# Rikorose/DeepFilterNet

Hardware: AMD Instinct MI355X
Metric: 48 kHz audio frames/sec (hop=480), DeepFilterNet3 enhance() (higher is better)
Workload: dtype f32 (storage and accumulation; GRU projections / recurrences, the fused DF-encoder convolutions and the pointwise halves of the ERB separable convolutions as fp16-split MFMAs: x = hi + lo in f16, hi*hi + hi*lo + lo*hi on v_mfma_f32_16x16x32_f16, ~2^-21 relative; see exact_fp32_ms_per_step); 1 GPU; DeepFilterNet3 (recalled shipped shape, conv_ch=64) enhance(pad=True), batch=256 clips x 10 s @48 kHz per GPU, 1002 STFT frames per clip; batch_per_gpu=256, global_batch=256, parallelism=clips sharded over 1 GPU(s); no collective, inputs_resident_in_hbm=True

## Files before the change

deepfilternet_amd/_lib.py:

```python
from __future__ import annotations

import ctypes as C
import os
from typing import Optional

import torch

_HERE = os.path.dirname(os.path.abspath(__file__))
DEFAULT_LIB = os.environ.get("DFX_LIBRARY") or os.path.join(_HERE, "csrc", "libdfx.so")

DFX_OK = 0
DFX_ERR_INVALID_ARG, DFX_ERR_UNSUPPORTED, DFX_ERR_HIP, DFX_ERR_NO_DEVICE, DFX_ERR_ALLOC = 1, 2, 3, 4, 5
_ERRNAMES = {1: "invalid argument", 2: "unsupported configuration", 3: "HIP runtime error", 4: "no HIP device",
             5: "allocation failed"}


class DfxError(RuntimeError):
    def __init__(self, code: int, msg: str):
        super().__init__(f"DF transform error: {msg} [{_ERRNAMES.get(code, code)}]")
        self.code = code


class ModelCfg(C.Structure):
    _fields_ = [(n, C.c_int32) for n in (
# ... 66 lines not shown
    "dfx_mf_filter": (_i, [_fp, _fp, _fp, _i, _i, _i, _i, _i, _i, _f, _f, _i64, _i64, _i, _i, _fp, _vp]),
    "dfx_pcm16_to_f32": (_i, [_vp, _i64, _fp, _vp]),
    "dfx_f32_to_pcm16": (_i, [_fp, _i64, _vp, _vp]),
    "dfx_resampler_create": (_i, [_i, _i, _i, C.c_double, _i, C.c_double, C.POINTER(_vp)]),
    "dfx_resampler_free": (None, [_vp]),
    "dfx_resampler_out_len": (_i64, [_vp, _i64]),
    "dfx_resampler_kernel": (_i, [_i, _i, _i, C.c_double, _i, C.c_double, C.POINTER(_i), C.POINTER(_i), C.POINTER(_i), _f32p, _i64]),
    "dfx_resample": (_i, [_vp, _fp, _i64, _i64, _i64, _fp, _i64, _vp]),
    "dfx_stream_create": (_i, [_vp, _vp, _i64, _i, C.POINTER(_vp)]),
    "dfx_stream_free": (None, [_vp]),
    "dfx_stream_reset": (_i, [_vp, _vp]),
    "dfx_stream_reset_streams": (_i, [_vp, C.POINTER(_i64), _i64, _vp]),
    "dfx_stream_frames": (_i, [_vp, C.POINTER(_i64)]),
    "dfx_stream_frame_length": (_i, [_vp]),
    "dfx_stream_delay_frames": (_i, [_vp]),
    "dfx_stream_set_atten_lim": (_i, [_vp, _f]),
    "dfx_stream_set_post_filter_beta": (_i, [_vp, _f]),
    "dfx_stream_set_channels": (_i, [_vp, _i, _i]),
    "dfx_stream_set_gating": (_i, [_vp, _i]),
    "dfx_stream_set_thresholds": (_i, [_vp, _f, _f, _f]),
    "dfx_stream_set_atten_lim_streams": (_i, [_vp, C.POINTER(_i64), _i64, C.POINTER(_f), _vp]),
    "dfx_stream_set_post_filter_beta_streams": (_i, [_vp, C.POINTER(_i64), _i64, C.POINTER(_f), _vp]),
    "dfx_stream_set_thresholds_streams": (_i, [_vp, C.POINTER(_i64), _i64, C.POINTER(_f), _vp]),
    "dfx_stream_get_settings": (_i, [_vp, C.POINTER(_f)]),
    "dfx_stream_process": (_i, [_vp, _fp, _i64, _fp, _fp, _vp]),
    "dfx_stream_set_pausable": (_i, [_vp, _i]),
    "dfx_stream_process_active": (_i, [_vp, _fp, _i64, _fp, _fp, _vp, _vp]),
    "dfx_stream_process_raw": (_i, [_vp, _fp, _fp, _fp, _vp, _fp, _vp]),
    "dfx_prof_kernel_count": (_i, []),
    "dfx_prof_kernel_name": (C.c_char_p, [_i]),
    "dfx_prof_enable": (_i, [C.c_uint32]),
    "dfx_prof_reset": (_i, []),
    "dfx_prof_read": (_i, [_i, C.POINTER(C.c_double), C.POINTER(_i64)]),
}

_LIB: Optional[C.CDLL] = None
_LIB_PATH: Optional[str] = None
_EMU = False


def _bind(lib: C.CDLL) -> None:
    missing = []
    for name, (res, args) in SIGNATURES.items():
        try:
            fn = getattr(lib, name)
        except AttributeError:
            missing.append(name)
            continue
        fn.restype, fn.argtypes = res, args
    if missing:
        raise RuntimeError(f"libdfx is missing symbols declared in include/dfx.h: {missing}")


def use_library(path: str) -> None:
    global _LIB, _LIB_PATH, _EMU
    lib = C.CDLL(path)
    _bind(lib)
    _LIB, _LIB_PATH = lib, path
    _EMU = bool(lib.dfx_is_emulator())


def lib() -> C.CDLL:
    if _LIB is None:
        if not os.path.exists(DEFAULT_LIB):
            from . import build as _build

# ... 81 lines not shown
```

deepfilternet_amd/csrc/dfx_common.h:

```cpp
#pragma once

#include "dfx_env.h"

#include <cstdarg>
#include <string>
#include <vector>

#include "dfx.h"

void dfx_set_error(const char *fmt, ...);
#define DFX_FAIL(code, ...)         \
    do {                            \
        dfx_set_error(__VA_ARGS__); \
        return (code);              \
    } while (0)
#define DFX_HIP(expr)                                                                                   \
    do {                                                                                                \
        hipError_t e__ = (expr);                                                                        \
        if (e__ != hipSuccess) DFX_FAIL(DFX_ERR_HIP, "%s failed: %s", #expr, hipGetErrorString(e__));   \
    } while (0)
#define DFX_LAUNCH_CHECK()                                                                              \
    do {                                                                                                \
        hipError_t e__ = hipGetLastError();                                                             \
        if (e__ != hipSuccess) DFX_FAIL(DFX_ERR_HIP, "kernel launch failed: %s", hipGetErrorString(e__)); \
    } while (0)
int dfx_require_device();

#define DFX_MAX_STAGES 12
struct DfxFftPlan {
    int N;
    int M;
    int nstage;
    int radix[DFX_MAX_STAGES];
};

struct dfx_bands {
    int nb = 0;
    int F = 0;
    std::vector<uint64_t> widths;
    int *d_start = nullptr;
    float *d_invw = nullptr;
// ... 81 lines not shown
```

deepfilternet_amd/csrc/dfx_gru_pair.h:

```cpp
#pragma once

#define DFX_GP_NW 4
#define DFX_GP_THREADS (64 * DFX_GP_NW)
#define DFX_GP_NS 2
#define DFX_GP_TILES (3 * DFX_GP_NS)
#define DFX_GP_NF (8 * DFX_GP_TILES)
#ifndef DFX_GP_FL
#define DFX_GP_FL 15
#endif
#define DFX_GP_FR (DFX_GP_NF - DFX_GP_FL)
#ifndef DFX_GP_PIN
#define DFX_GP_PIN 30
#endif
#ifndef DFX_GP_ABLATE
#define DFX_GP_ABLATE 0
#endif
#ifndef DFX_GP_TRACE
#define DFX_GP_TRACE 0
#endif
#if DFX_GP_TRACE
#define DFX_GP_TICK(i)                                                                  \
    do {                                                                                \
        unsigned long long now_;                                                        \
        asm volatile("s_memtime %0\n\ts_waitcnt lgkmcnt(0)" : "=s"(now_)::"memory");    \
        tk[i] += now_ - tlast;                                                          \
        tlast = now_;                                                                   \
    } while (0)
#else
#define DFX_GP_TICK(i) do { } while (0)
#endif
#define DFX_GP_ROWS 32
#define DFX_GP_SMEM_W ((size_t)DFX_GP_FL * DFX_GP_NW * 2 * 64 * 16)
#define DFX_GP_SMEM_H ((size_t)2 * DFX_GP_ROWS * DFX_GH_HROW * 2)
#define DFX_GP_SMEM (DFX_GP_SMEM_W + DFX_GP_SMEM_H + 64)
#define DFX_GP_POS_KC(f) ((f) / DFX_GP_TILES)
#define DFX_GP_POS_GATE(f) (((f) % DFX_GP_TILES) / DFX_GP_NS)
#define DFX_GP_POS_S(f) (((f) % DFX_GP_TILES) % DFX_GP_NS)
#define DFX_GP_POS_TILE(f) ((f) % DFX_GP_TILES)

struct DfxGpSched {
    int cls[DFX_GP_NF];
    int idx[DFX_GP_NF];
};
static constexpr DfxGpSched dfx_gp_make_sched() {
    DfxGpSched sc{};
    int nr = 0, nl = 0;
    for (int f = 0; f < DFX_GP_NF; ++f) {
        const bool lds = ((f + 1) * DFX_GP_FL / DFX_GP_NF) != (f * DFX_GP_FL / DFX_GP_NF);
        sc.cls[f] = lds ? 1 : 0;
        sc.idx[f] = lds ? nl++ : nr++;
    }
    return sc;
}

struct DfxGpSync {
    unsigned int *pflag = nullptr;
    unsigned int *pxcd = nullptr;
    unsigned int pbase = 0, tag = 0;
    int spin_limit = 1 << 22;
    unsigned int *err = nullptr;
    unsigned int *stat = nullptr;
    const unsigned int *ready = nullptr;
    unsigned int *done = nullptr;
    unsigned int base = 0;
    int K = 1;
    const int *tb = nullptr;
    unsigned long long *trace = nullptr;
    unsigned int *yprog = nullptr;
    const unsigned int *giprog[2] = {nullptr, nullptr};
    int sblk = 16, yblk = 16;
    unsigned int *xme = nullptr;
    const unsigned int *xprod[2] = {nullptr, nullptr};
    const unsigned int *xcons = nullptr;
    unsigned long long *ptrace = nullptr;
    int far = 0;
};

template <bool SEQ>
static __device__ __forceinline__ void dfx_gru_p2_run(const DfxGhArgs &A, int64_t pg, int half, const DfxGpSync &Y) {
    constexpr int H = 256, NF = DFX_GP_NF, HROW = DFX_GH_HROW, NW = DFX_GP_NW, NS = DFX_GP_NS, TILES = DFX_GP_TILES, ROWS = DFX_GP_ROWS;
    constexpr DfxGpSched SC = dfx_gp_make_sched();
    DFX_DYN_SMEM(unsigned char, smraw);
    dfx_h8 *wl = reinterpret_cast<dfx_h8 *>(smraw);
    uint16_t *h16 = reinterpret_cast<uint16_t *>(smraw + DFX_GP_SMEM_W);
    volatile int *sflag = reinterpret_cast<volatile int *>(smraw + DFX_GP_SMEM_W + DFX_GP_SMEM_H);
    const int tid = threadIdx.x, lane = tid & 63, wave = tid >> 6, q = lane >> 4, jl = lane & 15;
    const int64_t b0 = pg * ROWS;
    bool valid[2];
    int64_t brow[2];
#pragma unroll
    for (int n = 0; n < 2; ++n) {
        valid[n] = b0 + 16 * n + jl < A.B;
        brow[n] = valid[n] ? b0 + 16 * n + jl : A.B - 1;
    }
    const int ubase = 128 * half + 32 * wave;
    const dfx_h8 *wg = A.whf + lane;
#define DFX_GP_GIDX(f) (((((size_t)(8 * half + NS * wave + DFX_GP_POS_S(f))) * 8 + DFX_GP_POS_KC(f)) * 3 + DFX_GP_POS_GATE(f)) * 2 * 64)
    dfx_h8 wr[DFX_GP_FR][2];
    dfx_static_for<0, NF>([&](auto fc) {
        constexpr int f = decltype(fc)::value;
        if constexpr (SC.cls[f] == 0) {
            wr[SC.idx[f]][0] = wg[DFX_GP_GIDX(f)];
            wr[SC.idx[f]][1] = wg[DFX_GP_GIDX(f) + 64];
            if constexpr (SC.idx[f] < DFX_GP_PIN) {
                DFX_PIN_AGPR(wr[SC.idx[f]][0]);
                DFX_PIN_AGPR(wr[SC.idx[f]][1]);
            }
        } else {
            wl[((SC.idx[f] * NW + wave) * 2 + 0) * 64 + lane] = wg[DFX_GP_GIDX(f)];
            wl[((SC.idx[f] * NW + wave) * 2 + 1) * 64 + lane] = wg[DFX_GP_GIDX(f) + 64];
        }
    });
    float hp[2][NS][4];
    float4 bn[NS];
#pragma unroll
    for (int s = 0; s < NS; ++s) {
        bn[s] = *reinterpret_cast<const float4 *>(A.bhn + ubase + 16 * s + 4 * q);
#pragma unroll
        for (int n = 0; n < 2; ++n) hp[n][s][0] = hp[n][s][1] = hp[n][s][2] = hp[n][s][3] = 0.f;
    }
    auto put4 = [&](int row, int col, float v0, float v1, float v2, float v3) {
        const float v[4] = {v0, v1, v2, v3};
        uint16_t hh[4], hl[4];
#pragma unroll
        for (int r = 0; r < 4; ++r) {
            hh[r] = dfx_f32_to_f16_bits(v[r]);
            hl[r] = dfx_f32_to_f16_bits(v[r] - dfx_f16_bits_to_f32(hh[r]));
        }
        *reinterpret_cast<uint2 *>(h16 + ((size_t)0 * ROWS + row) * HROW + col) = make_uint2((uint32_t)hh[0] | ((uint32_t)hh[1] << 16), (uint32_t)hh[2] | ((uint32_t)hh[3] << 16));
        *reinterpret_cast<uint2 *>(h16 + ((size_t)1 * ROWS + row) * HROW + col) = make_uint2((uint32_t)hl[0] | ((uint32_t)hl[1] << 16), (uint32_t)hl[2] | ((uint32_t)hl[3] << 16));
    };
    for (int i = tid; i < (int)(DFX_GP_SMEM_H / 4); i += DFX_GP_THREADS) reinterpret_cast<uint32_t *>(h16)[i] = 0u;
    unsigned int *const fmine = Y.pflag + 16 * half;
    const unsigned int *const ftheirs = Y.pflag + 16 * (half ^ 1);
    bool dead = false;
    if (tid == 0) {
        const unsigned int me = Y.tag | (unsigned int)(dfx_xcc_id() + 1);
        __hip_atomic_store(Y.pxcd + half, me, __ATOMIC_RELAXED, __HIP_MEMORY_SCOPE_AGENT);
        if (Y.xme) __hip_atomic_store(Y.xme, me, __ATOMIC_RELAXED, __HIP_MEMORY_SCOPE_AGENT);
        unsigned int v;
        int spins = 0;
        while ((((v = __hip_atomic_load(Y.pxcd + (half ^ 1), __ATOMIC_RELAXED, __HIP_MEMORY_SCOPE_AGENT)) & ~15u) != Y.tag) || (v & 15u) == 0u) {
            if (++spins > Y.spin_limit) {
                dfx_raise(Y.err + 2);
                dead = true;
                break;
            }
            __builtin_amdgcn_s_sleep(2);
        }
        sflag[0] = (!dead && v == me && !Y.far) ? 1 : 0;
        sflag[1] = 0;
        if (Y.stat && half == 0 && v != me) __hip_atomic_fetch_add(Y.stat + 1, 1u, __ATOMIC_RELAXED, __HIP_MEMORY_SCOPE_AGENT);
    }
    __syncthreads();
    const bool light = sflag[0] != 0;
    const float *gp[2];
    float *yp[2];
    const float *ypo[4];
    const int prow = tid >> 3, pcol = 128 * (half ^ 1) + 4 * (tid & 7);
    {
        const int64_t r = b0 + prow < A.B ? b0 + prow : A.B - 1;
#pragma unroll
        for (int i = 0; i < 4; ++i) ypo[i] = A.y + r * A.T * H + pcol + 32 * i;
// ... 35 lines not shown
            }
            same = same && Y.xprod[i] && __hip_atomic_load(Y.xprod[i], __ATOMIC_RELAXED, __HIP_MEMORY_SCOPE_AGENT) == (Y.tag | (unsigned int)(dfx_xcc_id() + 1));
        }
        sflag[1] = same && !Y.far ? 1 : 0;
    };
#if DFX_GP_TRACE
    unsigned long long tk[12] = {0, 0, 0, 0, 0, 0, 0, 0, 0, 0, 0, 0}, tlast;
    asm volatile("s_memtime %0\n\ts_waitcnt lgkmcnt(0)" : "=s"(tlast)::"memory");
#endif
    const int nchunk = SEQ ? Y.K : 1;
    for (int ck = 0; ck < nchunk; ++ck) {
        const int64_t c0 = SEQ ? (int64_t)Y.tb[ck] : A.t0, c1 = SEQ ? (int64_t)Y.tb[ck + 1] : A.t1;
        if (SEQ) {
            if (tid == 0 && Y.trace) Y.trace[ck * 3 + 0] = wall_clock64();
            if (tid == 0 && !Y.giprog[0] && Y.ready) {
                const unsigned int want = Y.base + (unsigned int)ck + 1u;
                int spins = 0;
                while (!dead && (int)(__hip_atomic_load(Y.ready, __ATOMIC_RELAXED, __HIP_MEMORY_SCOPE_AGENT) - want) < 0) {
                    if (++spins > Y.spin_limit) {
                        dfx_raise(Y.err + 2);
                        dead = true;
                        break;
                    }
                    __builtin_amdgcn_s_sleep(8);
                }
            }
            if (tid == 0 && Y.giprog[0] && ck == 0) poll_gi(Y.sblk);
            __syncthreads();
            __builtin_amdgcn_fence(__ATOMIC_ACQUIRE, "agent");
            if (tid == 0 && Y.trace) Y.trace[ck * 3 + 1] = wall_clock64();
        }
        if (c1 > c0) load_gi(c0);
        for (int64_t t = c0; t < c1; ++t) {
            const unsigned char *hb = reinterpret_cast<const unsigned char *>(h16 + (size_t)jl * HROW + 8 * q);
            constexpr size_t HB_N = (size_t)16 * HROW * 2, HB_LO = (size_t)ROWS * HROW * 2, HB_KSTEP = 32 * 2;
            f32x4 acc[2][TILES];
#pragma unroll
            for (int n = 0; n < 2; ++n)
#pragma unroll
                for (int i = 0; i < TILES; ++i) acc[n][i] = f32x4{0.f, 0.f, 0.f, 0.f};
            dfx_h8 bh[2][2], bl[2][2];
#pragma unroll
            for (int n = 0; n < 2; ++n) {
                bh[0][n] = *reinterpret_cast<const dfx_h8 *>(hb + HB_N * n);
                bl[0][n] = *reinterpret_cast<const dfx_h8 *>(hb + HB_N * n + HB_LO);
            }
            dfx_h8 lhi[2][3], llo[2][3];
            dfx_static_for<0, 3>([&](auto ic) {
                constexpr int i = decltype(ic)::value;
                if constexpr (SC.cls[i] == 1) {
                    lhi[0][i] = wl[((SC.idx[i] * NW + wave) * 2 + 0) * 64 + lane];
                    llo[0][i] = wl[((SC.idx[i] * NW + wave) * 2 + 1) * 64 + lane];
                }
            });
            dfx_static_for<0, NF / 3>([&](auto gc) {
                constexpr int grp = decltype(gc)::value, f0 = 3 * grp;
                constexpr int kc = DFX_GP_POS_KC(f0);
                if constexpr (DFX_GP_POS_TILE(f0) == 0 && kc + 1 < 8) {
                    constexpr int kn = kc + 1;
#pragma unroll
                    for (int n = 0; n < 2; ++n) {
                        bh[kn & 1][n] = *reinterpret_cast<const dfx_h8 *>(hb + HB_N * n + HB_KSTEP * kn);
                        bl[kn & 1][n] = *reinterpret_cast<const dfx_h8 *>(hb + HB_N * n + HB_LO + HB_KSTEP * kn);
                    }
                }
                if constexpr (grp + 1 < NF / 3) {
                    dfx_static_for<0, 3>([&](auto ic) {
                        constexpr int i = decltype(ic)::value, f = f0 + 3 + i;
// ... 197 lines not shown
```

deepfilternet_amd/csrc/dfx_io.hip:

```cpp
#include <cmath>

#include "dfx_common.h"

#define DFX_RS_JT 16

struct dfx_resampler {
    int orig_sr = 0, new_sr = 0;
    int orig = 0, nw = 0, width = 0, K = 0, K4 = 0, nw_pad = 0;
    float *d_wt = nullptr;
    std::vector<float> w_host;
};

struct DfxRsArgs {
    int64_t B, T, x_stride, y_stride, out_len, frames;
    int orig, nw, nw_pad, width, K4, tn, fw, jw;
};

__global__ void __launch_bounds__(256) dfx_k_resample(const float *__restrict__ x, float *__restrict__ y, const float *__restrict__ wt,
                                                      DfxRsArgs A) {
    DFX_DYN_SMEM(float, xs);
    const int64_t tiles = (A.frames + A.tn - 1) / A.tn;
    const int64_t b = blockIdx.x / tiles;
    const int64_t n0 = (int64_t)(blockIdx.x - b * tiles) * A.tn;
    if (b >= A.B) return;
// ... 49 lines not shown
        out[i] = (float)in[i] * (1.0f / 32768.0f);
}
__global__ void dfx_k_f32_to_pcm16(const float *in, int64_t n, int16_t *out) {
    for (int64_t i = (int64_t)blockIdx.x * blockDim.x + threadIdx.x; i < n; i += (int64_t)gridDim.x * blockDim.x) {
        float v = in[i] * 32768.0f;
        v = v != v ? 0.f : fminf(fmaxf(v, -9.0e18f), 9.0e18f);
        out[i] = (int16_t)(uint16_t)(uint64_t)(int64_t)v;
    }
}

static unsigned io_grid(int64_t n) {
    const int64_t cap = (int64_t)dfx_env_num_cus() * 8, want = dfx_ceil_div(n, 256);
    return (unsigned)(want < cap ? (want > 0 ? want : 1) : cap);
}

extern "C" int dfx_pcm16_to_f32(const int16_t *pcm, int64_t n, float *out, void *stream) {
    if (n < 0) DFX_FAIL(DFX_ERR_INVALID_ARG, "dfx_pcm16_to_f32: bad arguments");
    if (int rc = dfx_require_device()) return rc;
    if (n == 0) return DFX_OK;
    if (!pcm || !out) DFX_FAIL(DFX_ERR_INVALID_ARG, "dfx_pcm16_to_f32: null buffer");
    DfxKScope ks(DFX_K_PCM, dfx_stream(stream));
    dfx_launch(dfx_k_pcm16_to_f32, dim3(io_grid(n)), dim3(256), 0, dfx_stream(stream), pcm, n, out);
    DFX_LAUNCH_CHECK();
    return DFX_OK;
}

extern "C" int dfx_f32_to_pcm16(const float *x, int64_t n, int16_t *out, void *stream) {
    if (n < 0) DFX_FAIL(DFX_ERR_INVALID_ARG, "dfx_f32_to_pcm16: bad arguments");
    if (int rc = dfx_require_device()) return rc;
    if (n == 0) return DFX_OK;
    if (!x || !out) DFX_FAIL(DFX_ERR_INVALID_ARG, "dfx_f32_to_pcm16: null buffer");
    DfxKScope ks(DFX_K_PCM, dfx_stream(stream));
    dfx_launch(dfx_k_f32_to_pcm16, dim3(io_grid(n)), dim3(256), 0, dfx_stream(stream), x, n, out);
    DFX_LAUNCH_CHECK();
    return DFX_OK;
}

static double bessel_i0(double x) {
    double sum = 1.0, term = 1.0;
    const double q = x * x / 4.0;
    for (int k = 1; k < 200; ++k) {
        term *= q / ((double)k * (double)k);
        sum += term;
        if (term < 1e-17 * sum) break;
    }
    return sum;
}

static int64_t gcd64(int64_t a, int64_t b) {
    while (b) {
        const int64_t t = a % b;
        a = b;
        b = t;
    }
    return a;
}

static int build_bank(dfx_resampler *r, int orig_sr, int new_sr, int lpw, double rolloff, int method, double beta) {
    if (orig_sr <= 0 || new_sr <= 0 || lpw <= 0 || rolloff <= 0.0 || rolloff > 1.0 || (method != 0 && method != 1))
        DFX_FAIL(DFX_ERR_INVALID_ARG, "dfx_resampler_create: bad arguments");
    const int64_t g = gcd64(orig_sr, new_sr);
    r->orig_sr = orig_sr, r->new_sr = new_sr;
    r->orig = (int)(orig_sr / g), r->nw = (int)(new_sr / g);
    const double base = (double)(r->orig < r->nw ? r->orig : r->nw) * rolloff;
    r->width = (int)std::ceil((double)lpw * r->orig / base);
    r->K = 2 * r->width + r->orig;
// ... 104 lines not shown
```

deepfilternet_amd/csrc/dfx_model.hip:

```cpp
#include "dfx_manifest.h"
#include "dfx_nn_kernels.h"

#include <cmath>
#include <functional>
#include <atomic>
#include <map>
#include <mutex>
#include <fcntl.h>
#include <sys/file.h>
#include <sys/stat.h>
#include <unistd.h>

static int check_cfg(const dfx_model_cfg *c) {
    if (!c) DFX_FAIL(DFX_ERR_INVALID_ARG, "null model cfg");
    if (c->conv_ch != 16 && c->conv_ch != 32 && c->conv_ch != 64)
        DFX_FAIL(DFX_ERR_UNSUPPORTED, "conv_ch=%d: the HIP kernels are instantiated for 16, 32, 64", c->conv_ch);
    if (c->emb_hidden_dim != 256 || c->df_hidden_dim != 256) DFX_FAIL(DFX_ERR_UNSUPPORTED, "GRU hidden size must be 256");
    if (c->nb_erb <= 0 || c->nb_erb % 8 || c->nb_erb > 64) DFX_FAIL(DFX_ERR_UNSUPPORTED, "nb_erb must be a multiple of 8, <= 64");
    if (c->nb_df <= 0 || c->nb_df % 2 || c->nb_df > c->fft_size / 2 + 1) DFX_FAIL(DFX_ERR_UNSUPPORTED, "nb_df must be even and <= F");
    if (c->df_order <= 0 || c->df_order > 16 || c->df_lookahead < 0 || c->df_lookahead >= c->df_order)
        DFX_FAIL(DFX_ERR_UNSUPPORTED, "need 0 <= df_lookahead < df_order <= 16");
    if (c->conv_lookahead < 0) DFX_FAIL(DFX_ERR_INVALID_ARG, "conv_lookahead < 0");
    if (c->emb_num_layers < 2 || c->df_num_layers < 1) DFX_FAIL(DFX_ERR_UNSUPPORTED, "emb_num_layers >= 2 and df_num_layers >= 1 required");
    if (c->df_pathway_kernel_size_t < 1 || c->df_pathway_kernel_size_t > 8) DFX_FAIL(DFX_ERR_UNSUPPORTED, "df_pathway_kernel_size_t must be 1..8");
// ... 1221 lines not shown
    w.gi = take(R * 768);
    w.xa2 = take(R * 256);
    w.xb2 = take(R * 256);
    w.gi2 = take(R * 768);
    w.demb = take(R * emb);
    w.d3 = take(R * (E / 4) * C);
    w.d2 = take(R * (E / 2) * C);
    w.d1 = take(R * E * C);
    w.mask = take(R * E);
    w.c0p = take(R * Fd * NO);
    w.xdf = take(R * 256);
    w.coefs = take(R * Fd * NO);
    w.lsnr = take(R);
    w.skp_e = take(c.emb_gru_skip_enc == DFX_SKIP_GROUPEDLINEAR ? R * emb : 0);
    w.skp_d = take(c.emb_gru_skip == DFX_SKIP_GROUPEDLINEAR ? R * emb : 0);
    const int nlayers = 1 + (c.emb_num_layers - 1) + c.df_num_layers;
    for (int l = 0; l < DFX_MAX_GRU_LAYERS; ++l) {
        const bool used = l < nlayers;
        w.pgi[l] = take(used ? R * 768 : 0);
        w.py[l] = take(used ? R * 256 : 0);
        w.ph[l] = take(used ? (B > 0 ? B : R) * 256 : 0);
    }
    w.total = off;
    return w;
}
}

extern "C" int dfx_model_workspace_bytes(const dfx_model *m, int64_t B, int64_t T, int64_t *bytes) {
    if (!m || !bytes || B < 0 || T < 0) DFX_FAIL(DFX_ERR_INVALID_ARG, "dfx_model_workspace_bytes: bad arguments");
    *bytes = (int64_t)(plan_ws(m->cfg, m->fuse_c0 && !m->c0_batch_unfused, B * T, B).total * sizeof(float)) + 256;
    return DFX_OK;
}

#include "dfx_model_launch.h"
#include "dfx_model_forward.h"
#include "dfx_model_stream.h"
#include "dfx_model_enhance.h"
```

deepfilternet_amd/csrc/dfx_nn_kernels.h:

```cpp
#pragma once

#include "dfx_common.h"

#include <type_traits>

#define DFX_ACT_NONE 0
#define DFX_ACT_RELU 1
#define DFX_ACT_TANH 2
#define DFX_ACT_SIGMOID 3

static __device__ __forceinline__ float dfx_sigmoid(float x) { return 1.f / (1.f + expf(-x)); }
static __device__ __forceinline__ float dfx_act(float v, int act) {
    if (act == DFX_ACT_RELU) return fmaxf(v, 0.f);
    if (act == DFX_ACT_TANH) return tanhf(v);
    if (act == DFX_ACT_SIGMOID) return dfx_sigmoid(v);
    return v;
}

template <int I, int N, typename F>
static __device__ __forceinline__ void dfx_static_for(F &&f) {
    if constexpr (I < N) {
        f(std::integral_constant<int, I>{});
        dfx_static_for<I + 1, N>(f);
    }
// ... 3884 lines not shown
    const dfx_h8 *wg = A.whf + lane;
#define DFX_GH_GIDX(f) (((((size_t)wave * NS + DFX_GH_POS_S(f)) * 8 + DFX_GH_POS_KC(f)) * 3 + DFX_GH_POS_GATE(f)) * 2 * 64)
    dfx_h8 wr[FR][2];
    dfx_static_for<0, NF>([&](auto fc) {
        constexpr int f = decltype(fc)::value;
        if constexpr (SC.cls[f] == 0) {
            wr[SC.idx[f]][0] = wg[DFX_GH_GIDX(f)];
            wr[SC.idx[f]][1] = wg[DFX_GH_GIDX(f) + 64];
            if constexpr (DFX_GH_PIN && !X32) {
                DFX_PIN_AGPR(wr[SC.idx[f]][0]);
                DFX_PIN_AGPR(wr[SC.idx[f]][1]);
            }
        } else if constexpr (SC.cls[f] == 1) {
            wl[((SC.idx[f] * NW + wave) * 2 + 0) * 64 + lane] = wg[DFX_GH_GIDX(f)];
            wl[((SC.idx[f] * NW + wave) * 2 + 1) * 64 + lane] = wg[DFX_GH_GIDX(f) + 64];
        }
    });
    float hp[NS][4];
    float4 bn[NS];
#pragma unroll
    for (int s = 0; s < NS; ++s) {
        const int u0 = UW * wave + 16 * s + 4 * q;
        bn[s] = *reinterpret_cast<const float4 *>(A.bhn + u0);
        float4 h0 = make_float4(0.f, 0.f, 0.f, 0.f);
        if (A.h_in) h0 = *reinterpret_cast<const float4 *>(A.h_in + brow * H + u0);
        hp[s][0] = h0.x, hp[s][1] = h0.y, hp[s][2] = h0.z, hp[s][3] = h0.w;
    }
    auto put_h16 = [&](int buf, int s) {
        if constexpr (X32) {
            *reinterpret_cast<float4 *>(h32 + ((size_t)buf * DFX_GH_ROWS + jl) * DFX_GH_HROW32 + UW * wave + 16 * s + 4 * q) =
                make_float4(hp[s][0], hp[s][1], hp[s][2], hp[s][3]);
            return;
        }
        uint16_t hh[4], hl[4];
#pragma unroll
        for (int r = 0; r < 4; ++r) {
            hh[r] = dfx_f32_to_f16_bits(hp[s][r]);
            hl[r] = dfx_f32_to_f16_bits(hp[s][r] - dfx_f16_bits_to_f32(hh[r]));
        }
        const int col = UW * wave + 16 * s + 4 * q;
        uint16_t *ph = h16 + ((size_t)(buf * 2 + 0) * DFX_GH_ROWS + jl) * HROW + col;
        uint16_t *pl = h16 + ((size_t)(buf * 2 + 1) * DFX_GH_ROWS + jl) * HROW + col;
        *reinterpret_cast<uint2 *>(ph) = make_uint2((uint32_t)hh[0] | ((uint32_t)hh[1] << 16), (uint32_t)hh[2] | ((uint32_t)hh[3] << 16));
        *reinterpret_cast<uint2 *>(pl) = make_uint2((uint32_t)hl[0] | ((uint32_t)hl[1] << 16), (uint32_t)hl[2] | ((uint32_t)hl[3] << 16));
    };
#pragma unroll
    for (int s = 0; s < NS; ++s) put_h16(0, s);
    __syncthreads();
    dfx_h8 ring[D][2];
    dfx_static_for<0, D>([&](auto dc) {
        constexpr int d = decltype(dc)::value;
        ring[d][0] = wg[DFX_GH_GIDX(SC.spos[d])];
        ring[d][1] = wg[DFX_GH_GIDX(SC.spos[d]) + 64];
    });
    const float *gp = A.gi + brow * A.T * (3 * H) + UW * wave + 4 * q;
    float *yp = A.y + brow * A.T * H + UW * wave + 4 * q;
    int cur = 0;
    float4 gv[3][NS];
#pragma unroll
    for (int g = 0; g < 3; ++g)
#pragma unroll
        for (int s = 0; s < NS; ++s) gv[g][s] = make_float4(0.1f, 0.2f, 0.3f, 0.4f);
    auto wait_gi = [&](int64_t upto) {
        if (tid == 0) {
            const unsigned int want = Y.pbase + (unsigned int)(upto < A.T ? upto : A.T);
            int spins = 0;
            while ((int)(__hip_atomic_load(Y.giprog, __ATOMIC_RELAXED, __HIP_MEMORY_SCOPE_AGENT) - want) < 0) {
                if (++spins > Y.spin_limit) {
                    dfx_raise(Y.err + 2);
                    break;
                }
                __builtin_amdgcn_s_sleep(2);
            }
        }
        __syncthreads();
        dfx_xcd_acquire(Y.x);
    };
// ... 567 lines not shown
```

deepfilternet_amd/csrc/env_hip/dfx_env.h:

```cpp
#pragma once

#include <hip/hip_runtime.h>

#include <cstdint>
#include <cstdio>
#include <cstdlib>
#include <cstring>
#include <utility>

typedef float f32x4 __attribute__((ext_vector_type(4)));
typedef float f32x2 __attribute__((ext_vector_type(2)));
typedef float f32x16 __attribute__((ext_vector_type(16)));

#define DFX_DYN_SMEM(T, name)                                                        \
    extern __shared__ __attribute__((aligned(16))) unsigned char dfx_dyn_smem_raw[]; \
    T *name = reinterpret_cast<T *>(dfx_dyn_smem_raw)

template <typename... KArgs, typename... Args>
static inline void dfx_launch(void (*kernel)(KArgs...), dim3 grid, dim3 block, size_t shmem, hipStream_t stream,
                              Args &&...args) {
    hipLaunchKernelGGL(kernel, grid, block, shmem, stream, static_cast<KArgs>(args)...);
}

static inline int dfx_env_num_cus() {
// ... 18 lines not shown
    return hipFuncSetAttribute(func, hipFuncAttributeMaxDynamicSharedMemorySize, (int)bytes);
}

static inline hipError_t dfx_env_err_words_alloc(unsigned int **host, unsigned int **dev, size_t bytes) {
    void *h = nullptr, *d = nullptr;
    hipError_t e = hipHostMalloc(&h, bytes, hipHostMallocMapped | hipHostMallocCoherent);
    if (e != hipSuccess) return e;
    memset(h, 0, bytes);
    e = hipHostGetDevicePointer(&d, h, 0);
    if (e != hipSuccess) {
        (void)hipHostFree(h);
        return e;
    }
    *host = static_cast<unsigned int *>(h), *dev = static_cast<unsigned int *>(d);
    return hipSuccess;
}
static inline void dfx_env_err_words_free(unsigned int *host) {
    if (host) (void)hipHostFree(host);
}
static __device__ __forceinline__ void dfx_raise(unsigned int *word) { __hip_atomic_store(word, 1u, __ATOMIC_RELAXED, __HIP_MEMORY_SCOPE_SYSTEM); }

typedef _Float16 dfx_h8 __attribute__((ext_vector_type(8)));
static __device__ __host__ __forceinline__ uint16_t dfx_f32_to_f16_bits(float x) {
    const _Float16 h = (_Float16)x;
    uint16_t b;
    __builtin_memcpy(&b, &h, 2);
    return b;
}
static __device__ __host__ __forceinline__ float dfx_f16_bits_to_f32(uint16_t b) {
    _Float16 h;
    __builtin_memcpy(&h, &b, 2);
    return (float)h;
}
typedef _Float16 dfx_h2v __attribute__((ext_vector_type(2)));
typedef float dfx_f2v __attribute__((ext_vector_type(2)));
static __device__ __forceinline__ void dfx_split8(const float *x, dfx_h8 &hi, dfx_h8 &lo) {
#pragma unroll
    for (int i = 0; i < 8; i += 2) {
        const dfx_f2v v = {x[i], x[i + 1]};
        const dfx_h2v h = __builtin_convertvector(v, dfx_h2v);
        const dfx_f2v r = v - __builtin_convertvector(h, dfx_f2v);
        const dfx_h2v l = __builtin_convertvector(r, dfx_h2v);
        hi[i] = h[0], hi[i + 1] = h[1];
        lo[i] = l[0], lo[i + 1] = l[1];
    }
}
#define DFX_H3_LIMIT 6.0e4f
static __device__ __forceinline__ void dfx_split8_g(const float *x, dfx_h8 &hi, dfx_h8 &lo, float &amax) {
#ifndef DFX_NO_H3_GUARD
    amax = fmaxf(amax, fmaxf(fmaxf(fmaxf(fabsf(x[0]), fabsf(x[1])), fmaxf(fabsf(x[2]), fabsf(x[3]))),
                             fmaxf(fmaxf(fabsf(x[4]), fabsf(x[5])), fmaxf(fabsf(x[6]), fabsf(x[7])))));
#endif
    dfx_split8(x, hi, lo);
}
static __device__ __forceinline__ f32x4 dfx_mfma_16x16x32_f16(dfx_h8 a, dfx_h8 b, f32x4 c) {
#ifdef DFX_MFMA_K16
    typedef _Float16 dfx_h4v __attribute__((ext_vector_type(4)));
    const dfx_h4v a0 = {a[0], a[1], a[2], a[3]}, a1 = {a[4], a[5], a[6], a[7]}, b0 = {b[0], b[1], b[2], b[3]}, b1 = {b[4], b[5], b[6], b[7]};
    c = __builtin_amdgcn_mfma_f32_16x16x16f16(a0, b0, c, 0, 0, 0);
    return __builtin_amdgcn_mfma_f32_16x16x16f16(a1, b1, c, 0, 0, 0);
#else
    return __builtin_amdgcn_mfma_f32_16x16x32_f16(a, b, c, 0, 0, 0);
#endif
}

static __device__ __forceinline__ float dfx_lane_gather4(float v, unsigned byte_addr) {
    return __builtin_bit_cast(float, __builtin_amdgcn_ds_bpermute((int)byte_addr, __builtin_bit_cast(int, v)));
}
#define DFX_MUL24(a, b) __mul24((a), (b))
#define DFX_OPAQUE(x) asm volatile("" : "+v"(x))
#define DFX_ASSUME(c) __builtin_assume(c)
#define DFX_PIN_AGPR(x) asm volatile("" : "+a"(x))
#define DFX_SCHED_BARRIER() __builtin_amdgcn_sched_barrier(0)
#define DFX_MFMA_GUARD()                         \
    do {                                         \
        __builtin_amdgcn_sched_barrier(0);       \
        asm volatile("s_nop 7");                 \
        __builtin_amdgcn_sched_barrier(0);       \
    } while (0)
#define DFX_VMEM_DRAIN() asm volatile("s_waitcnt vmcnt(0)" ::: "memory")
#define DFX_L1_INV() asm volatile("buffer_inv sc0" ::: "memory")
#define DFX_SCHED_GROUP(mask, n) __builtin_amdgcn_sched_group_barrier(mask, n, 0)
#ifdef DFX_WAVE_SYNC_WAIT
#define DFX_WAVE_SYNC()                                          \
// ... 22 lines not shown
```

include/dfx.h:

```cpp
#ifndef DFX_H
#define DFX_H

#include <stddef.h>
#include <stdint.h>

#ifdef __cplusplus
extern "C" {
#endif

#define DFX_OK 0
#define DFX_ERR_INVALID_ARG 1
#define DFX_ERR_UNSUPPORTED 2
#define DFX_ERR_HIP 3
#define DFX_ERR_NO_DEVICE 4
#define DFX_ERR_ALLOC 5

#define DFX_VERSION 200

int dfx_version(void);
const char *dfx_status_string(int status);
const char *dfx_last_error(void);
int dfx_device_count(void);
int dfx_is_emulator(void);

// ... 120 lines not shown
                                            void *stream);
int dfx_stream_set_thresholds_streams(dfx_stream_state *s, const int64_t *ids, int64_t count, const float *thr ,
                                      void *stream);
int dfx_stream_get_settings(const dfx_stream_state *s, float *out_host);
int dfx_stream_process(dfx_stream_state *s, const float *x, int64_t n_frames, float *y, float *lsnr, void *stream);
int dfx_stream_set_pausable(dfx_stream_state *s, int enable);
int dfx_stream_process_active(dfx_stream_state *s, const float *x, int64_t n_frames, float *y, float *lsnr,
                              const unsigned char *active, void *stream);
int dfx_stream_process_raw(dfx_stream_state *s, const float *spec, float *gains, float *coefs, unsigned char *stages, float *lsnr,
                           void *stream);

int dfx_mf_filter(const float *spec, const float *ifc, const float *mat, int op, int frame_size, int lookahead, int cholesky_decomp,
                  int inverse, int enforce_constraints, float eps, float dload, int64_t B, int64_t T, int F, int nb, float *out,
                  void *stream);

int dfx_pcm16_to_f32(const int16_t *pcm, int64_t n, float *out, void *stream);
int dfx_f32_to_pcm16(const float *x, int64_t n, int16_t *out, void *stream);
typedef struct dfx_resampler dfx_resampler;
int dfx_resampler_create(int orig_sr, int new_sr, int lowpass_filter_width, double rolloff, int method, double beta,
                         dfx_resampler **out);
void dfx_resampler_free(dfx_resampler *r);
int64_t dfx_resampler_out_len(const dfx_resampler *r, int64_t in_len);
int dfx_resampler_kernel(int orig_sr, int new_sr, int lowpass_filter_width, double rolloff, int method, double beta, int *phases,
                         int *taps, int *width, float *w_host , int64_t cap_floats);
int dfx_resample(const dfx_resampler *r, const float *x, int64_t B, int64_t T, int64_t x_stride, float *y, int64_t y_stride,
                 void *stream);

int dfx_prof_kernel_count(void);
const char *dfx_prof_kernel_name(int kernel_id);
int dfx_prof_enable(uint32_t kernel_mask);
int dfx_prof_reset(void);
int dfx_prof_read(int kernel_id, double *total_ms, int64_t *launches);

#ifdef __cplusplus
}
#endif
#endif
```

Measured before the change: 23.56 million frames/s.

## Split fp32 to f16 hi/lo pairs with packed mix-FMA asm and re-layout GRU hidden smem

Replaces the per-element f32->f16 hi/lo split with a packed inline-asm sequence (v_cvt_pk_f16_f32 plus v_fma_mixlo/mixhi) that produces two hi and two lo halves in three instructions, and uses v_max3 for the overflow guard's abs-max. The paired GRU kernel's hidden-state LDS buffer moves to a new swizzled 560-byte row layout, with the MFMA operand read offsets derived from it, presumably to reduce LDS bank conflicts. Self-test entry points are added to check the split and the offset function. The hand-written asm and the new layout risk subtle rounding or addressing mismatches.

New measurement: 23.64 million frames/s (median of 3 runs). No clear change (+0.3%).

```diff
diff --git a/deepfilternet_amd/_lib.py b/deepfilternet_amd/_lib.py
--- a/deepfilternet_amd/_lib.py
+++ b/deepfilternet_amd/_lib.py
@@ -122,6 +122,8 @@
     "dfx_prof_enable": (_i, [C.c_uint32]),
     "dfx_prof_reset": (_i, []),
     "dfx_prof_read": (_i, [_i, C.POINTER(C.c_double), C.POINTER(_i64)]),
+    "dfx_selftest_split": (_i, [_fp, _i64, _vp, _vp, _vp]),
+    "dfx_selftest_gru_h_offset": (_i64, [_i, _i, _i]),
 }
 
 _LIB: Optional[C.CDLL] = None
diff --git a/deepfilternet_amd/csrc/dfx_common.h b/deepfilternet_amd/csrc/dfx_common.h
--- a/deepfilternet_amd/csrc/dfx_common.h
+++ b/deepfilternet_amd/csrc/dfx_common.h
@@ -7,6 +7,14 @@
 #include <vector>
 
 #include "dfx.h"
+
+#ifndef DFX_ENV_SPLIT2
+static __device__ __forceinline__ void dfx_split2(float a, float b, uint32_t &hi_pk, uint32_t &lo_pk) {
+    const uint16_t ha = dfx_f32_to_f16_bits(a), hb = dfx_f32_to_f16_bits(b);
+    const uint16_t la = dfx_f32_to_f16_bits(a - dfx_f16_bits_to_f32(ha)), lb = dfx_f32_to_f16_bits(b - dfx_f16_bits_to_f32(hb));
+    hi_pk = (uint32_t)ha | ((uint32_t)hb << 16), lo_pk = (uint32_t)la | ((uint32_t)lb << 16);
+}
+#endif
 
 void dfx_set_error(const char *fmt, ...);
 #define DFX_FAIL(code, ...)         \
diff --git a/deepfilternet_amd/csrc/dfx_gru_pair.h b/deepfilternet_amd/csrc/dfx_gru_pair.h
--- a/deepfilternet_amd/csrc/dfx_gru_pair.h
+++ b/deepfilternet_amd/csrc/dfx_gru_pair.h
@@ -31,7 +31,12 @@
 #endif
 #define DFX_GP_ROWS 32
 #define DFX_GP_SMEM_W ((size_t)DFX_GP_FL * DFX_GP_NW * 2 * 64 * 16)
-#define DFX_GP_SMEM_H ((size_t)2 * DFX_GP_ROWS * DFX_GH_HROW * 2)
+#define DFX_GP_HROW_BYTES 560
+static constexpr int dfx_gp_h_offset(int row, int unit, int lo) {
+    const int kc = unit >> 5, q = (unit >> 3) & 3;
+    return (lo * DFX_GP_ROWS + row) * DFX_GP_HROW_BYTES + (16 * (q & 1) + (q >> 1) + 2 * kc) * 16 + (unit & 7) * 2;
+}
+#define DFX_GP_SMEM_H ((size_t)2 * DFX_GP_ROWS * DFX_GP_HROW_BYTES)
 #define DFX_GP_SMEM (DFX_GP_SMEM_W + DFX_GP_SMEM_H + 64)
 #define DFX_GP_POS_KC(f) ((f) / DFX_GP_TILES)
 #define DFX_GP_POS_GATE(f) (((f) % DFX_GP_TILES) / DFX_GP_NS)
@@ -78,11 +83,11 @@
 
 template <bool SEQ>
 static __device__ __forceinline__ void dfx_gru_p2_run(const DfxGhArgs &A, int64_t pg, int half, const DfxGpSync &Y) {
-    constexpr int H = 256, NF = DFX_GP_NF, HROW = DFX_GH_HROW, NW = DFX_GP_NW, NS = DFX_GP_NS, TILES = DFX_GP_TILES, ROWS = DFX_GP_ROWS;
+    constexpr int H = 256, NF = DFX_GP_NF, NW = DFX_GP_NW, NS = DFX_GP_NS, TILES = DFX_GP_TILES, ROWS = DFX_GP_ROWS;
     constexpr DfxGpSched SC = dfx_gp_make_sched();
     DFX_DYN_SMEM(unsigned char, smraw);
     dfx_h8 *wl = reinterpret_cast<dfx_h8 *>(smraw);
-    uint16_t *h16 = reinterpret_cast<uint16_t *>(smraw + DFX_GP_SMEM_W);
+    unsigned char *h16 = smraw + DFX_GP_SMEM_W;
     volatile int *sflag = reinterpret_cast<volatile int *>(smraw + DFX_GP_SMEM_W + DFX_GP_SMEM_H);
     const int tid = threadIdx.x, lane = tid & 63, wave = tid >> 6, q = lane >> 4, jl = lane & 15;
     const int64_t b0 = pg * ROWS;
@@ -120,15 +125,11 @@
         for (int n = 0; n < 2; ++n) hp[n][s][0] = hp[n][s][1] = hp[n][s][2] = hp[n][s][3] = 0.f;
     }
     auto put4 = [&](int row, int col, float v0, float v1, float v2, float v3) {
-        const float v[4] = {v0, v1, v2, v3};
-        uint16_t hh[4], hl[4];
-#pragma unroll
-        for (int r = 0; r < 4; ++r) {
-            hh[r] = dfx_f32_to_f16_bits(v[r]);
-            hl[r] = dfx_f32_to_f16_bits(v[r] - dfx_f16_bits_to_f32(hh[r]));
-        }
-        *reinterpret_cast<uint2 *>(h16 + ((size_t)0 * ROWS + row) * HROW + col) = make_uint2((uint32_t)hh[0] | ((uint32_t)hh[1] << 16), (uint32_t)hh[2] | ((uint32_t)hh[3] << 16));
-        *reinterpret_cast<uint2 *>(h16 + ((size_t)1 * ROWS + row) * HROW + col) = make_uint2((uint32_t)hl[0] | ((uint32_t)hl[1] << 16), (uint32_t)hl[2] | ((uint32_t)hl[3] << 16));
+        uint32_t h01, l01, h23, l23;
+        dfx_split2(v0, v1, h01, l01);
+        dfx_split2(v2, v3, h23, l23);
+        *reinterpret_cast<uint2 *>(h16 + dfx_gp_h_offset(row, col, 0)) = make_uint2(h01, h23);
+        *reinterpret_cast<uint2 *>(h16 + dfx_gp_h_offset(row, col, 1)) = make_uint2(l01, l23);
     };
     for (int i = tid; i < (int)(DFX_GP_SMEM_H / 4); i += DFX_GP_THREADS) reinterpret_cast<uint32_t *>(h16)[i] = 0u;
     unsigned int *const fmine = Y.pflag + 16 * half;
@@ -230,8 +231,9 @@
         }
         if (c1 > c0) load_gi(c0);
         for (int64_t t = c0; t < c1; ++t) {
-            const unsigned char *hb = reinterpret_cast<const unsigned char *>(h16 + (size_t)jl * HROW + 8 * q);
-            constexpr size_t HB_N = (size_t)16 * HROW * 2, HB_LO = (size_t)ROWS * HROW * 2, HB_KSTEP = 32 * 2;
+            const unsigned char *hb = h16 + dfx_gp_h_offset(jl, 8 * q, 0);
+            constexpr size_t HB_N = dfx_gp_h_offset(16, 0, 0), HB_LO = dfx_gp_h_offset(0, 0, 1), HB_KSTEP = dfx_gp_h_offset(0, 32, 0);
+            static_assert(dfx_gp_h_offset(31, 8 * 3 + 32 * 7, 1) == dfx_gp_h_offset(15, 8 * 3, 0) + HB_N + HB_LO + 7 * HB_KSTEP, "clip tile, half and k-chunk are plain strides");
             f32x4 acc[2][TILES];
 #pragma unroll
             for (int n = 0; n < 2; ++n)
diff --git a/deepfilternet_amd/csrc/dfx_io.hip b/deepfilternet_amd/csrc/dfx_io.hip
--- a/deepfilternet_amd/csrc/dfx_io.hip
+++ b/deepfilternet_amd/csrc/dfx_io.hip
@@ -105,6 +105,28 @@
     if (!x || !out) DFX_FAIL(DFX_ERR_INVALID_ARG, "dfx_f32_to_pcm16: null buffer");
     DfxKScope ks(DFX_K_PCM, dfx_stream(stream));
     dfx_launch(dfx_k_f32_to_pcm16, dim3(io_grid(n)), dim3(256), 0, dfx_stream(stream), x, n, out);
+    DFX_LAUNCH_CHECK();
+    return DFX_OK;
+}
+
+__global__ void dfx_k_selftest_split(const float *x, int64_t n8, dfx_h8 *hi, dfx_h8 *lo) {
+    for (int64_t i = (int64_t)blockIdx.x * blockDim.x + threadIdx.x; i < n8; i += (int64_t)gridDim.x * blockDim.x) {
+        float v[8];
+#pragma unroll
+        for (int j = 0; j < 8; ++j) v[j] = x[8 * i + j];
+        dfx_h8 h, l;
+        dfx_split8(v, h, l);
+        hi[i] = h, lo[i] = l;
+    }
+}
+
+extern "C" int dfx_selftest_split(const float *x, int64_t n, uint16_t *hi, uint16_t *lo, void *stream) {
+    if (n < 0 || n % 8 != 0) DFX_FAIL(DFX_ERR_INVALID_ARG, "dfx_selftest_split: n must be a non-negative multiple of 8");
+    if (int rc = dfx_require_device()) return rc;
+    if (n == 0) return DFX_OK;
+    if (!x || !hi || !lo || ((uintptr_t)hi | (uintptr_t)lo) % 16 != 0) DFX_FAIL(DFX_ERR_INVALID_ARG, "dfx_selftest_split: null or unaligned buffer");
+    dfx_launch(dfx_k_selftest_split, dim3(io_grid(n / 8)), dim3(256), 0, dfx_stream(stream), x, n / 8, reinterpret_cast<dfx_h8 *>(hi),
+               reinterpret_cast<dfx_h8 *>(lo));
     DFX_LAUNCH_CHECK();
     return DFX_OK;
 }
diff --git a/deepfilternet_amd/csrc/dfx_model.hip b/deepfilternet_amd/csrc/dfx_model.hip
--- a/deepfilternet_amd/csrc/dfx_model.hip
+++ b/deepfilternet_amd/csrc/dfx_model.hip
@@ -1277,6 +1277,12 @@
     return DFX_OK;
 }
 
+extern "C" int64_t dfx_selftest_gru_h_offset(int row, int unit, int lo) {
+    if (row < 0) return (int64_t)DFX_GP_SMEM_H;
+    if (row >= DFX_GP_ROWS || unit < 0 || unit >= 256 || lo < 0 || lo > 1) return -1;
+    return dfx_gp_h_offset(row, unit, lo);
+}
+
 #include "dfx_model_launch.h"
 #include "dfx_model_forward.h"
 #include "dfx_model_stream.h"
diff --git a/deepfilternet_amd/csrc/dfx_nn_kernels.h b/deepfilternet_amd/csrc/dfx_nn_kernels.h
--- a/deepfilternet_amd/csrc/dfx_nn_kernels.h
+++ b/deepfilternet_amd/csrc/dfx_nn_kernels.h
@@ -3940,17 +3940,14 @@
                 make_float4(hp[s][0], hp[s][1], hp[s][2], hp[s][3]);
             return;
         }
-        uint16_t hh[4], hl[4];
-#pragma unroll
-        for (int r = 0; r < 4; ++r) {
-            hh[r] = dfx_f32_to_f16_bits(hp[s][r]);
-            hl[r] = dfx_f32_to_f16_bits(hp[s][r] - dfx_f16_bits_to_f32(hh[r]));
-        }
+        uint32_t h01, l01, h23, l23;
+        dfx_split2(hp[s][0], hp[s][1], h01, l01);
+        dfx_split2(hp[s][2], hp[s][3], h23, l23);
         const int col = UW * wave + 16 * s + 4 * q;
         uint16_t *ph = h16 + ((size_t)(buf * 2 + 0) * DFX_GH_ROWS + jl) * HROW + col;
         uint16_t *pl = h16 + ((size_t)(buf * 2 + 1) * DFX_GH_ROWS + jl) * HROW + col;
-        *reinterpret_cast<uint2 *>(ph) = make_uint2((uint32_t)hh[0] | ((uint32_t)hh[1] << 16), (uint32_t)hh[2] | ((uint32_t)hh[3] << 16));
-        *reinterpret_cast<uint2 *>(pl) = make_uint2((uint32_t)hl[0] | ((uint32_t)hl[1] << 16), (uint32_t)hl[2] | ((uint32_t)hl[3] << 16));
+        *reinterpret_cast<uint2 *>(ph) = make_uint2(h01, h23);
+        *reinterpret_cast<uint2 *>(pl) = make_uint2(l01, l23);
     };
 #pragma unroll
     for (int s = 0; s < NS; ++s) put_h16(0, s);
diff --git a/deepfilternet_amd/csrc/env_hip/dfx_env.h b/deepfilternet_amd/csrc/env_hip/dfx_env.h
--- a/deepfilternet_amd/csrc/env_hip/dfx_env.h
+++ b/deepfilternet_amd/csrc/env_hip/dfx_env.h
@@ -74,24 +74,45 @@
     __builtin_memcpy(&h, &b, 2);
     return (float)h;
 }
+#define DFX_ENV_SPLIT2 1
 typedef _Float16 dfx_h2v __attribute__((ext_vector_type(2)));
 typedef float dfx_f2v __attribute__((ext_vector_type(2)));
+static __device__ __forceinline__ void dfx_split2(float a, float b, uint32_t &hi_pk, uint32_t &lo_pk) {
+#ifndef DFX_SPLIT_C
+    asm("v_cvt_pk_f16_f32 %0, %2, %3\n\t"
+        "v_fma_mixlo_f16 %1, %2, 1.0, -%0 op_sel_hi:[0,0,1]\n\t"
+        "v_fma_mixhi_f16 %1, %3, 1.0, -%0 op_sel:[0,0,1] op_sel_hi:[0,0,1]"
+        : "=&v"(hi_pk), "=&v"(lo_pk)
+        : "v"(a), "v"(b));
+#else
+    const dfx_f2v v = {a, b};
+    const dfx_h2v h = __builtin_convertvector(v, dfx_h2v);
+    const dfx_f2v r = v - __builtin_convertvector(h, dfx_f2v);
+    const dfx_h2v l = __builtin_convertvector(r, dfx_h2v);
+    hi_pk = __builtin_bit_cast(uint32_t, h), lo_pk = __builtin_bit_cast(uint32_t, l);
+#endif
+}
+typedef uint32_t dfx_u4v __attribute__((ext_vector_type(4)));
 static __device__ __forceinline__ void dfx_split8(const float *x, dfx_h8 &hi, dfx_h8 &lo) {
+    dfx_u4v h, l;
 #pragma unroll
-    for (int i = 0; i < 8; i += 2) {
-        const dfx_f2v v = {x[i], x[i + 1]};
-        const dfx_h2v h = __builtin_convertvector(v, dfx_h2v);
-        const dfx_f2v r = v - __builtin_convertvector(h, dfx_f2v);
-        const dfx_h2v l = __builtin_convertvector(r, dfx_h2v);
-        hi[i] = h[0], hi[i + 1] = h[1];
-        lo[i] = l[0], lo[i + 1] = l[1];
+    for (int i = 0; i < 4; ++i) {
+        uint32_t hp, lp;
+        dfx_split2(x[2 * i], x[2 * i + 1], hp, lp);
+        h[i] = hp, l[i] = lp;
     }
+    hi = __builtin_bit_cast(dfx_h8, h), lo = __builtin_bit_cast(dfx_h8, l);
 }
 #define DFX_H3_LIMIT 6.0e4f
 static __device__ __forceinline__ void dfx_split8_g(const float *x, dfx_h8 &hi, dfx_h8 &lo, float &amax) {
 #ifndef DFX_NO_H3_GUARD
+#ifndef DFX_SPLIT_C
+#pragma unroll
+    for (int i = 0; i < 8; i += 2) asm("v_max3_f32 %0, |%1|, |%2|, %0" : "+v"(amax) : "v"(x[i]), "v"(x[i + 1]));
+#else
     amax = fmaxf(amax, fmaxf(fmaxf(fmaxf(fabsf(x[0]), fabsf(x[1])), fmaxf(fabsf(x[2]), fabsf(x[3]))),
                              fmaxf(fmaxf(fabsf(x[4]), fabsf(x[5])), fmaxf(fabsf(x[6]), fabsf(x[7])))));
+#endif
 #endif
     dfx_split8(x, hi, lo);
 }
diff --git a/include/dfx.h b/include/dfx.h
--- a/include/dfx.h
+++ b/include/dfx.h
@@ -176,6 +176,9 @@
 int dfx_prof_reset(void);
 int dfx_prof_read(int kernel_id, double *total_ms, int64_t *launches);
 
+int dfx_selftest_split(const float *x, int64_t n, uint16_t *hi, uint16_t *lo, void *stream);
+int64_t dfx_selftest_gru_h_offset(int row, int unit, int lo);
+
 #ifdef __cplusplus
 }
 #endif
```
